# emolch/kiwi

Hardware: AMD Instinct MI355X
Metric: trial-source misfit evals/s (higher is better)
Workload: dtype f32

## Files before the change

### kiwi_amd/csrc/kiwi_accum.hip

```cpp
#include "kiwi_accum_api.hpp"

#if KIWI_ARITH == 0
#define KIWI_ARITH_NS exact
#elif KIWI_ARITH == 1
#define KIWI_ARITH_NS fused
#else
#error "KIWI_ARITH: 0 (exact) or 1 (fused)"
#endif

namespace kiwi {
namespace KIWI_ARITH_NS {

#include "kiwi_accum.inc"

#define KIWI_COMMON_ARGS a.G, a.span, a.pitch, a.recs, a.cent_ofs, a.isrc0, a.nrec, a.recv, a.syn, a.syn_stride

#if KIWI_FAMILY == 1
void launch_direct(const AccumArgs &a, dim3 grid)
{
    if (a.ng == 10) hipLaunchKernelGGL(accumulate_kernel<10>, grid, dim3(256), 0, a.stream, KIWI_COMMON_ARGS, a.synrow);
    else            hipLaunchKernelGGL(accumulate_kernel<8>, grid, dim3(256), 0, a.stream, KIWI_COMMON_ARGS, a.synrow);
}
#endif

// ... 22 lines not shown
    } else {
        if (T == 64) grouped_t<8, 64>(a, grid, ntiles, runs, pairsel, mate, mate4);
        else if (T == 128) grouped_t<8, 128>(a, grid, ntiles, runs, pairsel, mate, mate4);
        else grouped_t<8, 256>(a, grid, ntiles, runs, pairsel, mate, mate4);
    }
}
#endif

#if KIWI_FAMILY == 3
template <int NG, int NS, bool COMPACT, bool PLAN>
static void multi_t(const AccumArgs &a, dim3 grid, int ntiles, const int *mate, const int *wider)
{
    if (a.fuse) hipLaunchKernelGGL((accumulate_multi_kernel<NG, true, NS, COMPACT, PLAN>), grid, dim3(256), 0, a.stream, KIWI_COMMON_ARGS, ntiles, a.tab, a.coefs, a.fp,
                                   a.pairflag, mate, wider, a.plan, a.plan_ofs);
    else        hipLaunchKernelGGL((accumulate_multi_kernel<NG, false, NS, COMPACT, PLAN>), grid, dim3(256), 0, a.stream, KIWI_COMMON_ARGS, ntiles, a.tab, a.coefs, a.fp,
                                   a.pairflag, mate, wider, a.plan, a.plan_ofs);
}
template <int NG, int NS>
static void multi_c(const AccumArgs &a, dim3 grid, int ntiles, const int *mate, const int *wider)
{
    if (a.compact && a.plan) multi_t<NG, NS, true, true>(a, grid, ntiles, mate, wider);
    else if (a.compact) multi_t<NG, NS, true, false>(a, grid, ntiles, mate, wider);
    else multi_t<NG, NS, false, false>(a, grid, ntiles, mate, wider);
}
void launch_multi(const AccumArgs &a, dim3 grid, int NS, int ntiles, const int *mate, const int *wider)
{
    if (a.ng == 10) { if (NS == 4) multi_c<10, 4>(a, grid, ntiles, mate, wider); else multi_c<10, 2>(a, grid, ntiles, mate, wider); }
    else            { if (NS == 4) multi_c<8, 4>(a, grid, ntiles, mate, wider); else multi_c<8, 2>(a, grid, ntiles, mate, wider); }
}
void launch_multi_plan(const AccumArgs &a, int NS, int ngroups, const int *mate, const int *wider, PlanSrc *plan)
{
    const dim3 grid((unsigned)ngroups, (unsigned)((a.nrec + 63) / 64));
    if (NS == 4) hipLaunchKernelGGL(multi_plan_kernel<4>, grid, dim3(64), 0, a.stream, a.recs, a.cent_ofs, a.isrc0, a.nrec, a.recv, a.tab, a.pairflag, mate, wider,
                                    a.plan_ofs, (int4 *)plan);
    else         hipLaunchKernelGGL(multi_plan_kernel<2>, grid, dim3(64), 0, a.stream, a.recs, a.cent_ofs, a.isrc0, a.nrec, a.recv, a.tab, a.pairflag, mate, wider,
                                    a.plan_ofs, (int4 *)plan);
}
#endif

#if KIWI_FAMILY == 4
template <int NG, bool COMPACT>
static void cell_t(const AccumArgs &a, dim3 grid, int ntiles, bool per_wave)
{
#define KIWI_C(KERNEL) hipLaunchKernelGGL(KERNEL, grid, dim3(256), 0, a.stream, KIWI_COMMON_ARGS, ntiles, a.tab, a.coefs, a.fp, a.pairflag, a.synrow, \
                                          a.fam_ofs, a.fam_list)
    if (per_wave) { if (a.fuse) KIWI_C((accumulate_cellw_kernel<NG, true, COMPACT>)); else KIWI_C((accumulate_cellw_kernel<NG, false, COMPACT>)); }
    else          { if (a.fuse) KIWI_C((accumulate_cell_kernel<NG, 256, 2, 0, true, COMPACT>)); else KIWI_C((accumulate_cell_kernel<NG, 256, 2, 0, false, COMPACT>)); }
#undef KIWI_C
}
template <int NG>
static void cell_c(const AccumArgs &a, dim3 grid, int ntiles, bool per_wave)
{
    if (a.compact) cell_t<NG, true>(a, grid, ntiles, per_wave); else cell_t<NG, false>(a, grid, ntiles, per_wave);
}
void launch_cell(const AccumArgs &a, dim3 grid, int ntiles) { if (a.ng == 10) cell_c<10>(a, grid, ntiles, false); else cell_c<8>(a, grid, ntiles, false); }
void launch_cellw(const AccumArgs &a, dim3 grid, int ntiles) { if (a.ng == 10) cell_c<10>(a, grid, ntiles, true); else cell_c<8>(a, grid, ntiles, true); }
int cellw_range() { return kCellwRange; }
#endif

}
}
```

### kiwi_amd/csrc/kiwi_accum.inc

```


typedef float f4u __attribute__((ext_vector_type(4), aligned(4)));
typedef float f2u __attribute__((ext_vector_type(2), aligned(4)));

#if defined(KIWI_EXPLICIT_FMA)
#ifndef KIWI_CELLW_AHEAD
#define KIWI_CELLW_AHEAD 3
#endif
template <class V> __device__ __forceinline__ V kiwi_mad(V acc, float w, V v)
{
    V ws;
    for (int k = 0; k < (int)(sizeof(V) / sizeof(float)); k++) ws[k] = w;
    return __builtin_elementwise_fma(ws, v, acc);
}
template <class V> __device__ __forceinline__ V kiwi_madv(V acc, V w, V v) { return __builtin_elementwise_fma(w, v, acc); }
#else
template <class V> __device__ __forceinline__ V kiwi_mad(V acc, float w, V v) { return acc + w * v; }
template <class V> __device__ __forceinline__ V kiwi_madv(V acc, V w, V v) { return acc + w * v; }
#endif

typedef int v4i_t __attribute__((ext_vector_type(4)));
typedef int v2i_t __attribute__((ext_vector_type(2)));
__device__ __forceinline__ __amdgpu_buffer_rsrc_t gf_rsrc(const float *base)
{
// ... 788 lines not shown
        if constexpr (i < nH1) {
            t1[0] = t1[0] + c1 * s2a<i>(H); t1[0] = t1[0] + c2 * s2a<i>(L);
            t1[1] = t1[1] + c1 * s2b<i>(H); t1[1] = t1[1] + c2 * s2b<i>(L);
        } else if constexpr (i < nH1 + 2) {
            t2[0] = t2[0] + c1 * s2a<i>(H); t2[0] = t2[0] + c2 * s2a<i>(L);
            t2[1] = t2[1] + c1 * s2b<i>(H); t2[1] = t2[1] + c2 * s2b<i>(L);
        } else {
            dz[0] = dz[0] + c1 * s2a<i>(H); dz[0] = dz[0] + c2 * s2a<i>(L);
            dz[1] = dz[1] + c1 * s2b<i>(H); dz[1] = dz[1] + c2 * s2b<i>(L);
        }
        if constexpr (i == nH1 + 1) {
#pragma unroll
            for (int k = 0; k < 2; k++) {
                if (ROT) {
                    ar1[k] = ar1[k] + cl * t1[k] - sl * t2[k];
                    ar2[k] = ar2[k] + cl * t2[k] + sl * t1[k];
                } else {
                    ar1[k] = t1[k]; ar2[k] = t2[k];
                }
            }
        }
    });
}

template <int NG>
__device__ __forceinline__ typename Set2Sel<NG>::type make_set2(f2v &a0, f2v &a1, f2v &a2, f2v &a3, f2v &a4, f2v &a5, f2v &a6, f2v &a7, f2v &a8, f2v &a9,
                                                                f2v &b0, f2v &b1, f2v &b2, f2v &b3, f2v &b4, f2v &b5, f2v &b6, f2v &b7, f2v &b8, f2v &b9)
{
    if constexpr (NG == 10) return Set2_10{ a0, a1, a2, a3, a4, a5, a6, a7, a8, a9, b0, b1, b2, b3, b4, b5, b6, b7, b8, b9 };
    else return Set2_8{ a0, a1, a2, a3, a4, a5, a6, a7, b0, b1, b2, b3, b4, b5, b6, b7 };
}

#include "kiwi_apply_asm.inc"
__device__ __forceinline__ int coef_warm(const float *p)
{
    int d;
    asm volatile("s_load_dword %0, %1, 0x0\n\ts_load_dword %0, %1, 0x40\n\ts_load_dword %0, %1, 0x80\n\ts_load_dword %0, %1, 0xc0\n\t"
                 "s_load_dword %0, %1, 0x100\n\ts_load_dword %0, %1, 0x140\n\ts_load_dword %0, %1, 0x180\n\ts_load_dword %0, %1, 0x1c0"
                 : "=&s"(d) : "s"(p) : "memory");
    return d;
}
#if KIWI_ARITH == 1
#define KIWI_APPLY_ASM(NGV, KV, RV) apply_group_asm_##NGV##_k##KV##_##RV##_fused
#else
#define KIWI_APPLY_ASM(NGV, KV, RV) apply_group_asm_##NGV##_k##KV##_##RV##_exact
#endif

template <int NG, int T, bool FUSE, bool RUNS, bool COMPACT >
__global__ __launch_bounds__(T) __attribute__((amdgpu_waves_per_eu(3))) void accumulate_grouped_kernel(
    const float *__restrict__ G, const int2 *__restrict__ span, int pitch,
    const GeoRec *__restrict__ recs, const int *__restrict__ cent_ofs, int isrc0, int nrec,
    const RecvDev *__restrict__ recv, float *__restrict__ syn, size_t syn_stride, int ntiles,
    const int *__restrict__ tab, const float *__restrict__ coefs, const int *__restrict__ run_first, FuseParams fp,
    const int *__restrict__ pairflag ,
    int pairsel ,
    const int *__restrict__ mate, const int *__restrict__ mate4 ,
    const int *__restrict__ synrow ,
    const int *__restrict__ fam_ofs, const int *__restrict__ fam_list )
{
    constexpr bool compact = COMPACT;
    constexpr int TILE = 4 * T;
    constexpr int LDS_TILE = TILE + kHalo;
    __shared__ __attribute__((aligned(16))) float tiles[NG][LDS_TILE];
    const int s = RUNS ? run_first[blockIdx.x] : (int)blockIdx.x;
    const int s_end = RUNS ? run_first[blockIdx.x + 1] : s + 1;
    const bool multi = RUNS && s_end - s > 1;
    const int tile = blockIdx.y % ntiles, r = blockIdx.y / ntiles;
    const RecvDev &rv = recv[r];
    if (!rv.enabled) return;
    if (tile * TILE >= rv.wlen) return;
    if (pairsel == 1 && cell_pair(rv, pairflag, s, nrec, r)) return;
    if (pairsel == 3 && (multi_taken_fwd<4>(rv, pairflag, mate4, s, nrec, r) || multi_taken_fwd<2>(rv, pairflag, mate, s, nrec, r))) return;
    if (synrow && !multi && synrow[s] != s) return;
    const int tid = threadIdx.x;
    const int lane = tid & 63;
    const int t_tile0 = rv.wbeg + tile * TILE;
    const int cb = cent_ofs[isrc0], c0 = cent_ofs[isrc0 + s], nc = cent_ofs[isrc0 + s + 1] - c0;
    const GeoRec *__restrict__ rc = recs + ((size_t)(c0 - cb) * nrec + (size_t)r * nc);
// ... 456 lines not shown
#pragma unroll
            for (int s = 0; s < NS; s++)
                if (only < 0 || only == s) one_finish<true>(v[i], tile0 + s * SET, LDS_TILE, comp(i), p, gw[s]);
        }
        if (i + DEPTH < N && (i + DEPTH < N - 1 || last_ok)) issue(i + DEPTH);
    }
    if (whalo) {
#pragma unroll
        for (int s = 0; s < NS; s++)
            if (only < 0 || only == s) halo_finish<true>(hact, hv, tile0 + s * SET, LDS_TILE, hig, hph, gw[s]);
    }
}


__device__ __forceinline__ int smax_u(int a, int b) { int r; asm("s_max_i32 %0, %1, %2" : "=s"(r) : "s"(a), "s"(b) : "scc"); return r; }
__device__ __forceinline__ int smin_u(int a, int b) { int r; asm("s_min_i32 %0, %1, %2" : "=s"(r) : "s"(a), "s"(b) : "scc"); return r; }

template <int NS>
__device__ __forceinline__ bool multi_taken(const RecvDev &rv, const int *__restrict__ pairflag, const int *__restrict__ mate,
                                            int s, int nrec, int r)
{
    if (!mate) return false;
    const int a = s - s % NS;
    if (!mate[a / NS] || !rv.need_h || !rv.has_d) return false;
    int f = 0;
#pragma unroll
    for (int i = 0; i < NS; i++) f |= pairflag[(size_t)(a + i) * nrec + r];
    return f == 0;
}

template <int NS>
__global__ __launch_bounds__(64) void multi_plan_kernel(const GeoRec *__restrict__ recs, const int *__restrict__ cent_ofs, int isrc0, int nrec,
    const RecvDev *__restrict__ recv, const int *__restrict__ off4, const int *__restrict__ pairflag, const int *__restrict__ mate,
    const int *__restrict__ mate_wider, const int *__restrict__ plan_ofs, int4 *__restrict__ plan)
{
    constexpr int TILE = 1024 / NS, LDS_TILE = TILE + kHalo;
    const int k = (int)blockIdx.x, s0 = NS * k, r = (int)(blockIdx.y * 64 + threadIdx.x);
    if (r >= nrec) return;
    const RecvDev &rv = recv[r];
    if (!rv.enabled) return;
    if (!multi_taken<NS>(rv, pairflag, mate, s0, nrec, r)) return;
    if constexpr (NS == 2) { if (multi_taken<4>(rv, pairflag, mate_wider, s0, nrec, r)) return; }
    const int cb = cent_ofs[isrc0];
    const int nc = cent_ofs[isrc0 + s0 + 1] - cent_ofs[isrc0 + s0];
    const size_t pbeg = (size_t)plan_ofs[k], pend = (size_t)plan_ofs[k + 1];
    size_t pi = pbeg + (size_t)r;
    for (int c = 0; c < nc && pi < pend; pi += (size_t)nrec) {
        const GeoRec *h[NS];
        int smaxs[NS], smins[NS], npos = 0;
        bool shared = true, same_rows = true;
#pragma unroll
        for (int i = 0; i < NS; i++) {
            h[i] = recs + ((size_t)(cent_ofs[isrc0 + s0 + i] - cb) * nrec + (size_t)r * nc + c);
            smaxs[i] = h[i]->ishift + ((h[i]->pad >> 8) & 0xff);
            smins[i] = h[i]->ishift - ((h[i]->pad >> 16) & 0xff);
            npos = max(npos, TILE + (smaxs[i] - smins[i]) + 8);
            if (i > 0) {
                same_rows = same_rows && h[i]->row[0] == h[0]->row[0] && h[i]->row[1] == h[0]->row[1] && h[i]->row[2] == h[0]->row[2] && h[i]->row[3] == h[0]->row[3];
                shared = shared && smaxs[i] == smaxs[0];
            }
        }
        shared = shared && same_rows;
        if (same_rows && !shared) {
            int smax_c = smaxs[0], smin_c = smins[0];
#pragma unroll
            for (int i = 1; i < NS; i++) { smax_c = max(smax_c, smaxs[i]); smin_c = min(smin_c, smins[i]); }
            if (TILE + (smax_c - smin_c) + 8 <= LDS_TILE) {
                shared = true;
                npos = TILE + (smax_c - smin_c) + 8;
#pragma unroll
                for (int i = 0; i < NS; i++) smaxs[i] = smax_c;
            }
        }
        const int glen = h[0]->pad & 0xff;
        int4 *__restrict__ out = plan + pi * (kPlanStride / 16);
#pragma unroll
        for (int i = 0; i < NS; i++) {
            const int4 o = *(const int4 *)(off4 + ((size_t)(cent_ofs[isrc0 + s0 + i] - cb) * nrec + (size_t)r * nc + c) * 4);
            const int head = (h[i]->flags & 0xffff) | (glen << 16) | ((shared ? 1 : 0) << 23) | ((npos - TILE) << 24);
            out[4 * i + 0] = make_int4(h[i]->row[0], h[i]->row[1], h[i]->row[2], h[i]->row[3]);
            out[4 * i + 1] = o;
            out[4 * i + 2] = make_int4(__float_as_int(h[i]->w[0]), __float_as_int(h[i]->w[1]), __float_as_int(h[i]->w[2]), __float_as_int(h[i]->w[3]));
            out[4 * i + 3] = make_int4(smaxs[i], head, __float_as_int(h[i]->cl), __float_as_int(h[i]->sl));
        }
        if (glen < 1) break;
        c += glen;
    }
}

typedef const __attribute__((address_space(4))) v4i_t *plan_cptr;
template <int NS>
__device__ __forceinline__ int plan_warm(size_t p)
{
    int d;
    if constexpr (NS == 4)
        asm volatile("s_load_dword %0, %1, 0x0\n\ts_load_dword %0, %1, 0x40\n\ts_load_dword %0, %1, 0x80\n\ts_load_dword %0, %1, 0xc0" : "=&s"(d) : "s"(p) : "memory");
    else
        asm volatile("s_load_dword %0, %1, 0x0\n\ts_load_dword %0, %1, 0x40" : "=&s"(d) : "s"(p) : "memory");
    return d;
}

template <int NG, bool FUSE, int NS, bool COMPACT ,
          bool PLAN >
__global__ __launch_bounds__(256) __attribute__((amdgpu_waves_per_eu(3))) void accumulate_multi_kernel(
    const float *__restrict__ G, const int2 *__restrict__ span, int pitch,
    const GeoRec *__restrict__ recs, const int *__restrict__ cent_ofs, int isrc0, int nrec,
    const RecvDev *__restrict__ recv, float *__restrict__ syn, size_t syn_stride, int ntiles,
    const int *__restrict__ tab, const float *__restrict__ coefs, FuseParams fp, const int *__restrict__ pairflag, const int *__restrict__ mate,
    const int *__restrict__ mate_wider ,
    const PlanSrc *__restrict__ plan, const int *__restrict__ plan_ofs )
{
    constexpr bool compact = COMPACT;
    static_assert(NS == 2 || NS == 4, "sources per workgroup");
    static_assert(!PLAN || COMPACT, "plans hold compact descriptors");
    constexpr int TILE = 1024 / NS, LDS_TILE = TILE + kHalo, K = LDS_TILE / 64, WPS = 4 / NS;
    constexpr int SET = multi_set_stride<NG, NS>();
    __shared__ __attribute__((aligned(16))) float tiles[NS * SET];
// ... 94 lines not shown
            }
        }
        }
        const int glen = PLAN ? glen_p : (g[0].pad & 0xff);
        const int cend = c + glen;
        int smax = smaxs[0];
        if constexpr (PLAN) smax = plan4(64 * sh + 48).x;
        else {
#pragma unroll
            for (int i = 1; i < NS; i++) if (sh == i) smax = smaxs[i];
        }
        int flags = 0, ishv = 0, warm_ = 0, pwarm_ = 0;
        float gcl = 0.f, gsl = 0.f;
        const float *__restrict__ coef_grp = nullptr;
        auto shadow = [&]() {
            if constexpr (PLAN) {
#pragma unroll
                for (int i = 0; i < NS; i++) {
                    const v4i_t w = plan4(64 * i + 32);
                    g[i].w[0] = __int_as_float(w.x); g[i].w[1] = __int_as_float(w.y); g[i].w[2] = __int_as_float(w.z); g[i].w[3] = __int_as_float(w.w);
                }
                const v4i_t me = plan4(64 * sh + 48);
                flags = me.y & 0xffff; gcl = __int_as_float(me.z); gsl = __int_as_float(me.w);
                if (c + glen < nc) pwarm_ = plan_warm<NS>(pcur + (size_t)(unsigned)pstep);
            } else {
#pragma unroll
            for (int i = 0; i < NS; i++) { g[i].w[0] = REC_F(cur[i], 4); g[i].w[1] = REC_F(cur[i], 5); g[i].w[2] = REC_F(cur[i], 6); g[i].w[3] = REC_F(cur[i], 7); }
            int curme = cur[0];
#pragma unroll
            for (int i = 1; i < NS; i++) if (sh == i) curme = cur[i];
            flags = REC_I(curme, 18);
            gcl = REC_F(curme, 16); gsl = REC_F(curme, 17);
            }
            if (lane < glen) ishv = rc[c + lane].ishift;
            const size_t crow = (base_me + c) * kCoefLine;
            const unsigned clo = __builtin_amdgcn_readfirstlane((unsigned)crow), chi = __builtin_amdgcn_readfirstlane((unsigned)(crow >> 32));
            coef_grp = coefs + (((size_t)chi << 32) | clo);
            if constexpr (NG == 10) warm_ = coef_warm(coef_grp);
        };
        auto noshadow = []() {};
#define KIWI_MULTI_BUILD(DESC, I0, ONLY, NPOS, SHADOW) do { \
            const int jb_ = t_tile0 - smaxs[I0] - 1;       \
            const float *__restrict__ Gg = G + (size_t)g[I0].row[0] * (size_t)pitch; \
            const bool fast = (DESC).fast(jb_, LDS_TILE, pitch, lane, NG); \
            const bool hact = hq < 16 * NG && hph < (NPOS); \
            const bool whalo = __builtin_amdgcn_ballot_w64(hact) != 0ull; \
            if (fast) multi_build<NG, true, NS>(&tiles[0], wv, lane, tid, jb_, Gg, pitch, DESC, g, ONLY, hact, whalo, hig, hph, SHADOW); \
            else      multi_build<NG, false, NS>(&tiles[0], wv, lane, tid, jb_, Gg, pitch, DESC, g, ONLY, hact, whalo, hig, hph, SHADOW); } while (0)
        __builtin_amdgcn_s_setprio(1);
        if constexpr (PLAN) {
            if (shared) KIWI_MULTI_BUILD(dp, 0, -1, npos, shadow);
            else {
                KIWI_MULTI_BUILD(dp, 0, 0, npos, shadow);
#pragma unroll
                for (int i = 1; i < NS; i++) {
                    const v4i_t rw = plan4(64 * i), of = plan4(64 * i + 16);
                    smaxs[i] = plan4(64 * i + 48).x;
                    g[i].row[0] = rw.x;
                    const DescPlan di{ { 0, (rw.y - rw.x) * pitch, (rw.z - rw.x) * pitch, (rw.w - rw.x) * pitch }, { of.x, of.y, of.z, of.w }, pitch, hoff };
                    KIWI_MULTI_BUILD(di, i, i, npos, noshadow);
                }
            }
            asm volatile("" :: "s"(pwarm_));
            pcur += (size_t)(unsigned)pstep;
        } else {
        if (shared) KIWI_MULTI_BUILD((DescLanes{ ta, tb }), 0, -1, npos, shadow);
        else {
            KIWI_MULTI_BUILD((DescLanes{ ta, tb }), 0, 0, npos, shadow);
#pragma unroll
            for (int i = 1; i < NS; i++) {
                int tai, tbi;
                if constexpr (compact) desc_expand(off4_load(tab_of(i), c, lane), cur[i], lane, pitch, tai, tbi);
                else { tai = tab_of(i)[(size_t)c * 128 + lane]; tbi = tab_of(i)[(size_t)c * 128 + 64 + lane]; }
                g[i].row[0] = REC_I(cur[i], 0);
                KIWI_MULTI_BUILD((DescLanes{ tai, tbi }), i, i, npos, noshadow);
            }
        }
#pragma unroll
        for (int i = 0; i < NS; i++) cur[i] = rec_load(recs_of(i), cend, nc, lane);
        if (cend < nc) {
            if constexpr (compact) ta = off4_load(tab_of(0), cend, lane);
            else { ta = tab_of(0)[(size_t)cend * 128 + lane]; tb = tab_of(0)[(size_t)cend * 128 + 64 + lane]; }
        }
        }
#undef KIWI_MULTI_BUILD
        __syncthreads();
        __builtin_amdgcn_s_setprio(0);
        {
            const unsigned abase = (unsigned)(size_t)(lds_cfp)&tiles[sh * SET + u0];
            if constexpr (NG == 10 || NG == 8) {
                asm volatile("" :: "s"(warm_));
                const float gcl_u = __int_as_float(__builtin_amdgcn_readfirstlane(__float_as_int(gcl))), gsl_u = __int_as_float(__builtin_amdgcn_readfirstlane(__float_as_int(gsl)));
                const size_t cg_ = (size_t)coef_grp;
                const float *__restrict__ coef_u = (const float *)(((size_t)(unsigned)__builtin_amdgcn_readfirstlane((int)(cg_ >> 32)) << 32) | (unsigned)__builtin_amdgcn_readfirstlane((int)cg_));
                const int n = cend - c;
#define KIWI_ASM_ARGS ar1[0], ar1[1], ar2[0], ar2[1], dz[0], dz[1], abase, ishv, smax, n, coef_u, gcl_u, gsl_u
                if constexpr (NG == 10) {
                    if (flags & 2) { if constexpr (K == 5) KIWI_APPLY_ASM(10, 5, rot)(KIWI_ASM_ARGS); else KIWI_APPLY_ASM(10, 9, rot)(KIWI_ASM_ARGS); }
                    else           { if constexpr (K == 5) KIWI_APPLY_ASM(10, 5, plain)(KIWI_ASM_ARGS); else KIWI_APPLY_ASM(10, 9, plain)(KIWI_ASM_ARGS); }
                } else {
                    if (flags & 2) { if constexpr (K == 5) KIWI_APPLY_ASM(8, 5, rot)(KIWI_ASM_ARGS); else KIWI_APPLY_ASM(8, 9, rot)(KIWI_ASM_ARGS); }
                    else           { if constexpr (K == 5) KIWI_APPLY_ASM(8, 5, plain)(KIWI_ASM_ARGS); else KIWI_APPLY_ASM(8, 9, plain)(KIWI_ASM_ARGS); }
                }
#undef KIWI_ASM_ARGS
            } else {
            int cc = c, eprev = 0;
            bool have = false;
#define KIWI_C2STEP(LL, HH, RV, CC) do { \
                const int e = smax - __builtin_amdgcn_readlane(ishv, (CC) - c);        \
                const int d = have ? eprev - e : 0x7fff; \
                carry2_apply<NG, RV, K>(ar1, ar2, dz, LL, HH, abase + 4u * (unsigned)e, d, d, coef_grp + (size_t)((CC) - c) * kCoefLine, gcl, gsl); \
                have = true; eprev = e; } while (0)
            if (flags & 2) {
                set2_dead(X); set2_dead(Y);
                for (; cc + 1 < cend; cc += 2) { KIWI_C2STEP(X, Y, true, cc); KIWI_C2STEP(Y, X, true, cc + 1); }
                if (cc < cend) KIWI_C2STEP(X, Y, true, cc);
            } else {
                set2_dead(X); set2_dead(Y);
                for (; cc + 1 < cend; cc += 2) { KIWI_C2STEP(X, Y, false, cc); KIWI_C2STEP(Y, X, false, cc + 1); }
                if (cc < cend) KIWI_C2STEP(X, Y, false, cc);
            }
#undef KIWI_C2STEP
            }
        }
        c = cend;
    }
    {
        const int js = s0 + sh;
        const int tl = tile * TILE + u0;
        if (!FUSE && tl >= rv.wlen) return;
        float *__restrict__ so = syn + (size_t)js * syn_stride + tl;
        float mom = 0.f;
        if constexpr (FUSE) mom = fp.moment[fp.isrc0 + js];
        const bool whole = tile * TILE + TILE <= rv.wlen;
        for (int k = 0; k < rv.ncomp; k++) {
            f2v o01, o23;
            out4(rv.comp[k], rv.sign[k], rv.cl0, rv.sl0, ar1, ar2, dz, o01, o23);
// ... 585 lines not shown
```

### kiwi_amd/csrc/kiwi_accum_api.hpp

```cpp
#pragma once
#include "kiwi_common.hpp"

namespace kiwi {

struct AccumArgs {
    hipStream_t stream;
    int ng;
    bool fuse;
    const float *G; const int2 *span; int pitch;
    const GeoRec *recs; const int *cent_ofs; int isrc0, nrec;
    const RecvDev *recv; float *syn; size_t syn_stride;
    const int *tab; const float *coefs; FuseParams fp;
    const int *pairflag, *synrow, *fam_ofs, *fam_list;
    int compact;
    const PlanSrc *plan = nullptr;
    const int *plan_ofs = nullptr;
};

#define KIWI_ACCUM_LAUNCHERS                                                                                                      \
                                                                 \
    void launch_direct(const AccumArgs &a, dim3 grid);                                                                            \
                  \
    void launch_grouped(const AccumArgs &a, dim3 grid, int T, int ntiles, const int *runs, int pairsel, const int *mate,          \
                        const int *mate4);                                                                                        \
                                                     \
    void launch_multi(const AccumArgs &a, dim3 grid, int NS, int ntiles, const int *mate, const int *mate_wider);                \
                \
    void launch_multi_plan(const AccumArgs &a, int NS, int ngroups, const int *mate, const int *mate_wider, PlanSrc *plan);      \
        \
    void launch_cell(const AccumArgs &a, dim3 grid, int ntiles);                                                                  \
    void launch_cellw(const AccumArgs &a, dim3 grid, int ntiles);                                                                 \
                               \
    int cellw_range();

namespace exact { KIWI_ACCUM_LAUNCHERS }
namespace fused { KIWI_ACCUM_LAUNCHERS }
#undef KIWI_ACCUM_LAUNCHERS

}
```

### kiwi_amd/csrc/kiwi_common.hpp

```cpp
#pragma once
#include <hip/hip_runtime.h>
#include <type_traits>

namespace kiwi {

constexpr int kRowPad = 32;
constexpr int kTile = 1024;
constexpr int kMaxComp = 5;
constexpr int kHalo = 64;
constexpr int kMaxGroup = 64;

struct GeoRec {
    int   row[4];
    float w[4];
    int   ishift;
    float wfrac;
    float f[6];
    float cl, sl;
    int   flags;
    int   pad;
};
static_assert(sizeof(GeoRec) == 80, "GeoRec layout");

struct GfMeta {
// ... 36 lines not shown
    int ntrans_max;
    int fl_lo, fl_ns, refxofs;
    int untapered, rf0, rf1, vertical;
    int spankind;
};

struct FftPair {
    long long fft_ofs;
    long long spec_ofs;
    int ntrans;
    int specofs;
    int filtofs;
    int slot;
};
static_assert(sizeof(FftPair) == 32, "FftPair layout");

struct ShakeRec {
    int slot[3];
    int np;
    int untapered;
    int rec;
};

constexpr int kCoefLine = 20;
struct PlanSrc {
    int   row[4];
    int   o[4];
    float w[4];
    int   smax;
    int   head;
    float cl, sl;
};
static_assert(sizeof(PlanSrc) == 64, "PlanSrc layout");
constexpr int kPlanStride = 256;
template <int NG> __host__ __device__ constexpr int coef_wl(int a) { return 2 * a; }
template <int NG> __host__ __device__ constexpr int coef_wr(int a) { return 2 * a + 1; }

constexpr int kSpanInts = 8;
__device__ __forceinline__ void strip_span(const int *__restrict__ sp, int kind, int &lo, int &hi)
{
    if (kind == 3) { lo = sp[4]; hi = sp[5]; return; }
    if (kind == 0) { lo = sp[0]; hi = sp[1]; return; }
    if (kind == 1) { lo = sp[2]; hi = sp[3]; return; }
    lo = min(sp[0], sp[2]); hi = max(sp[1], sp[3]);
}

struct EvalParams {
    int bilinear, xus, zus;
    int nrec;
    int isrc0;
    int cellmode;
    int nogaps;
};

__device__ __forceinline__ bool cell_pair(const RecvDev &rv, const int *__restrict__ pairflag, int s, int nrec, int r)
{
    return rv.need_h && rv.has_d && !(pairflag[(size_t)s * nrec + r] & 3);
}

template <int NS>
__device__ __forceinline__ bool multi_taken_fwd(const RecvDev &rv, const int *__restrict__ pairflag, const int *__restrict__ mate,
                                                int s, int nrec, int r)
{
    if (!mate) return false;
    const int a = s - s % NS;
    if (!mate[a / NS] || !rv.need_h || !rv.has_d) return false;
// ... 36 lines not shown
```

### kiwi_amd/csrc/kiwi_hip.hip

```cpp
#include "../../include/kiwi_hip.h"
#include "kiwi_host.hpp"
#include "kiwi_host_eikonal.hpp"
#include "kiwi_host_lm.hpp"
#include "kiwi_geometry.hpp"
#include "kiwi_misfit.hpp"
#include "kiwi_accum_api.hpp"
#include "kiwi_fmm_device.hpp"

#include <hip/hip_runtime.h>
#include <hipfft/hipfft.h>
#include <algorithm>
#include <array>
#include <map>
#include <tuple>
#include <cstdio>
#include <cstdlib>
#include <cstring>
#include <string>
#include <vector>
#include <stdexcept>
#include <omp.h>
#include <chrono>
#include <condition_variable>
#include <deque>
// ... 140 lines not shown
    std::vector<RecvDev> recv_h;
    std::vector<float> norm_h;
    std::vector<float> reft_h;
    DevBuf<RecvDev> recv_d;
    DevBuf<CompDev> comps_d;
    DevBuf<float> reft_d, tw_d, norm_d;
    DevBuf<int> recfirst_d;
    int max_wlen = 0;

    int nsrc = 0;
    std::vector<int> cent_ofs;
    float max_risetime = 0.f;
    DevBuf<float> cent_d, moment_d, risetime_d;
    DevBuf<int> centofs_d;
    std::vector<int> src_status;
    bool any_failed = false;
    DevBuf<int> status_d;
    std::vector<int> same_as;
    bool any_same = false;
    DevBuf<int> synrow_d, famofs_d, famlist_d;
    int dedupe_enabled = 1;
    std::vector<unsigned long long> geo_hash;
    std::vector<kiwi_hip_ctx *> mates;
    int cpu_share = 1;
    std::vector<unsigned long long> struct_hash;
    std::vector<int> ngroups;
    std::vector<unsigned char> group_lens;
    std::vector<int> first_shift;
    std::vector<float> src_ends;
    DevBuf<int> mate_d, mate4_d;
    DevBuf<int> planofs_d;
    DevBuf<int4> plan_d;
    int multi_plan = 1;
    int duo = 4;
    std::vector<char> single_group;
    DevBuf<int> runfirst_d;
    int share_runs = 1, max_run = 64;
    int fuse_enabled = 1;
    bool fuse_now = false;
    DevBuf<double> fusepart_d;

    DevBuf<float> misfit_d, global_d;
    DevBuf<GeoRec> recs_d;
    DevBuf<int> tab_d;
    DevBuf<int> off4_d;
    DevBuf<float> coef_d;
    DevBuf<int> pairflag_d;
    DevBuf<float> syn_d, proc_d;
    bool floating = false;
    int max_ns = 1;
    DevBuf<float> refx_d, vt_d, partial_d;
    DevBuf<int> fshift_d;
    int last_isrc0 = 0, last_nsrc = 0, last_chunk0 = 0, last_chunkn = 0;
    std::vector<char> evaluated;
    int last_proc_which = 0;
    int group_threads_env = 0;
    int group_threads = 128;
    int accum_mode = 0;
    int cell_mode = -1;
    int cell_wave = 1;
    int arith = KIWI_ARITH_EXACT;
    double points_per_centroid = 0.0;
    int keep_which = 0;
    int proc_chunk0 = 0, proc_chunkn = 0, proc_which_held = 0;
    size_t chunk_bytes_limit = (size_t)16 << 30;
    float outer_ms[3] = { 0.f, 0.f, 0.f };
// ... 908 lines not shown
                            c->plan_d.ensure((np + 1) * (kPlanStride / 16), &c->dev_bytes);
                            HIPCHECK(hipMemcpyAsync(c->planofs_d.p, po, (n4 + n2 + 2) * sizeof(int), hipMemcpyHostToDevice, c->stream));
                            if (std::getenv("KIWI_HIP_POISON")) HIPCHECK(hipMemsetAsync(c->plan_d.p, 0x7f, (np + 1) * kPlanStride, c->stream));
                            planned = true;
                        }
                    }
                    HIPCHECK(hipEventRecord(c->mate_event, c->stream));
                }
            }
            const int ntiles_q = (c->max_wlen + 255) / 256;
            dim3 ggrid(gx, (unsigned)(ntiles * nrec));
            dim3 dgrid((unsigned)((nsrc + 1) / 2), (unsigned)(ntiles_p * nrec)), qgrid((unsigned)((nsrc + 3) / 4), (unsigned)(ntiles_q * nrec));
            dim3 cgrid((unsigned)nsrc, (unsigned)(ntiles_c * nrec));
            if (fuse) {
                const int nparts = cell ? std::max(ntiles * (T / 64), ntiles_c * (Tc / 64)) : (duo ? std::max({ ntiles * (T / 64), ntiles_p * 2, ntiles_q }) : ntiles * (T / 64));
                c->fusepart_d.ensure((size_t)nsrc * c->nmis * nparts, &c->dev_bytes);
                if (cell || duo) HIPCHECK(hipMemsetAsync(c->fusepart_d.p, 0, (size_t)nsrc * c->nmis * nparts * sizeof(double), c->stream));
                aa.fp = FuseParams{ c->reft_d.p, c->tw_d.p, c->moment_d.p, c->fusepart_d.p, c->method, c->syn_factor, c->nmis, nparts, isrc0 };
                fuse_nparts = nparts;
            }
            fuse_T = T; fuse_tile = 4 * T; fuse_ntiles = ntiles; fuse_all = cell || duo;
            aa.pairflag = (cell || duo) ? c->pairflag_d.p : (const int *)nullptr;
            if (cell) {
                static const bool cell_fused = [] { const char *e = std::getenv("KIWI_HIP_CELL_FUSED"); return !e || std::atoi(e) != 0; }();
                if (c->cell_wave) { if (fusedar && cell_fused) fused::launch_cellw(aa, cgrid, ntiles_c); else exact::launch_cellw(aa, cgrid, ntiles_c); }
                else exact::launch_cell(aa, cgrid, ntiles_c);
            }
            const int *m2p = any2 ? c->mate_d.p : (const int *)nullptr, *m4p = any4 ? c->mate4_d.p : (const int *)nullptr;
            AccumArgs aa4 = aa, aa2 = aa;
            if (planned) {
                const size_t n4 = (size_t)(nsrc + 3) / 4;
                aa4.plan = (const PlanSrc *)c->plan_d.p; aa4.plan_ofs = c->planofs_d.p;
                aa2.plan = (const PlanSrc *)(c->plan_d.p + plan_n4 * (kPlanStride / 16)); aa2.plan_ofs = c->planofs_d.p + n4 + 1;
                if (any4) { if (fusedar) fused::launch_multi_plan(aa4, 4, (int)qgrid.x, m4p, nullptr, (PlanSrc *)aa4.plan); else exact::launch_multi_plan(aa4, 4, (int)qgrid.x, m4p, nullptr, (PlanSrc *)aa4.plan); }
                if (any2) { if (fusedar) fused::launch_multi_plan(aa2, 2, (int)dgrid.x, m2p, m4p, (PlanSrc *)aa2.plan); else exact::launch_multi_plan(aa2, 2, (int)dgrid.x, m2p, m4p, (PlanSrc *)aa2.plan); }
            }
            if (any4) { if (fusedar) fused::launch_multi(aa4, qgrid, 4, ntiles_q, m4p, nullptr); else exact::launch_multi(aa4, qgrid, 4, ntiles_q, m4p, nullptr); }
            if (any2) { if (fusedar) fused::launch_multi(aa2, dgrid, 2, ntiles_p, m2p, m4p); else exact::launch_multi(aa2, dgrid, 2, ntiles_p, m2p, m4p); }
            const int pairsel = cell ? 1 : (duo ? 3 : 0);
            if (fusedar) fused::launch_grouped(aa, ggrid, T, ntiles, runs, pairsel, m2p, m4p);
            else         exact::launch_grouped(aa, ggrid, T, ntiles, runs, pairsel, m2p, m4p);
        }
    }
    record(c, 1, e2);
    if (c->any_untapered) {
        c->synspan_d.ensure((size_t)nsrc * c->nmis * 2, &c->dev_bytes);
        hipLaunchKernelGGL(synspan_kernel, dim3((unsigned)c->nmis, (unsigned)nsrc), dim3(256), 0, c->stream, c->syn_d.p, c->syn_stride, c->comps_d.p,
                           c->risetime_d.p + isrc0, c->gm.dt, c->nmis, spansrc, nrec, synrow, c->synspan_d.p);
    }
    if (c->untapered_fft) {
        const size_t np = (size_t)nsrc * c->nmis;
        c->ntr_d.ensure(np, &c->dev_bytes);
        pin_ensure(c->ntr_pin, c->ntr_pin_n, np);
        hipLaunchKernelGGL(fft_size_kernel, dim3((unsigned)((np + 255) / 256)), dim3(256), 0, c->stream, spansrc, c->comps_d.p, c->nmis,
                           nsrc, nrec, c->risetime_d.p + isrc0, c->gm.dt, c->ntr_d.p, (const int *)c->synspan_d.p);
        HIPCHECK(hipMemcpyAsync(c->ntr_pin, c->ntr_d.p, np * sizeof(int), hipMemcpyDeviceToHost, c->stream));
        HIPCHECK(hipEventRecord(c->size_event, c->stream));
    }
    if (c->fft_needed) layout_fft_chunk(c, isrc0, nsrc);
    {
        const bool spectral = (c->method == KIWI_AMPSPEC_L2NORM || c->method == KIWI_AMPSPEC_L1NORM);
        const int fl_method = c->method == KIWI_FLOATING_L2NORM ? KIWI_L2NORM : KIWI_L1NORM;
        const int td_method = spectral ? KIWI_L2NORM : (c->floating ? fl_method : c->method);
        const int fft_mode = !c->fft_needed ? 0 : (spectral ? 3 : 1);
        MisfitParams mp{ td_method, c->gm.dt, c->syn_factor, c->nmis, isrc0, proc_which == 3 ? 2 : proc_which, fft_mode, nsrc,
                         c->floating ? 1 : 0 };
        if (c->floating) {
            c->vt_d.ensure((size_t)nsrc * c->syn_stride, &c->dev_bytes);
// ... 170 lines not shown
#pragma unroll
        for (int k = 0; k < 8; k++) v[k] = __builtin_nontemporal_load(p + i + 256 * k);
#pragma unroll
        for (int k = 0; k < 8; k++) { x ^= v[k].x; y ^= v[k].y; z ^= v[k].z; w ^= v[k].w; }
    }
    for (; i < b; i += 256) { const read_u4 v = p[i]; x ^= v.x; y ^= v.y; z ^= v.z; w ^= v.w; }
    if ((x ^ y ^ z ^ w) == 0x9e3779b9u) sink[blockIdx.x] = x;
}

extern "C" {

int kiwi_hip_init(int device, kiwi_hip_ctx **out)
{
    kmp_set_blocktime(0);
    kiwi_hip_ctx *c = nullptr;
    try {
        int ndev = 0;
        hipError_t e = hipGetDeviceCount(&ndev);
        if (e != hipSuccess || ndev <= 0)
            return fail(nullptr, std::string("no HIP device available: ") + hipGetErrorString(e));
        if (device < 0 || device >= ndev) return fail(nullptr, "device index out of range");
        HIPCHECK(hipSetDevice(device));
        c = new kiwi_hip_ctx();
        c->device = device;
        HIPCHECK(hipStreamCreateWithFlags(&c->stream, hipStreamNonBlocking));
        if (const char *m = std::getenv("KIWI_HIP_GROUP_THREADS")) {
            const int v = std::atoi(m);
            if (v == 64 || v == 128 || v == 256) { c->group_threads = v; c->group_threads_env = 1; }
        }
        if (const char *m = std::getenv("KIWI_HIP_ACCUM")) c->accum_mode = (std::strcmp(m, "direct") == 0) ? 1 : 0;
        if (const char *m = std::getenv("KIWI_HIP_FUSE")) c->fuse_enabled = std::atoi(m);
        if (const char *m = std::getenv("KIWI_HIP_DUO")) { const int v = std::atoi(m); c->duo = v >= 4 ? 4 : (v >= 1 ? 2 : 0); }
        if (const char *m = std::getenv("KIWI_HIP_MULTI_PLAN")) c->multi_plan = std::atoi(m) ? 1 : 0;
        if (const char *m = std::getenv("KIWI_HIP_CELL")) c->cell_mode = std::atoi(m) ? 1 : 0;
        if (const char *m = std::getenv("KIWI_HIP_DEDUPE")) c->dedupe_enabled = std::atoi(m);
        if (const char *m = std::getenv("KIWI_HIP_FUSED_FFT")) c->fused_fft = std::atoi(m) != 0;
        if (const char *m = std::getenv("KIWI_HIP_ARITH")) {
            if (std::strcmp(m, "fused") == 0 || std::strcmp(m, "fma") == 0) c->arith = KIWI_ARITH_FUSED;
            else if (std::strcmp(m, "exact") != 0) throw std::runtime_error("KIWI_HIP_ARITH: exact or fused");
        }
        if (const char *m = std::getenv("KIWI_HIP_CELL_WAVE")) c->cell_wave = std::atoi(m) ? 1 : 0;
        if (const char *m = std::getenv("KIWI_HIP_COMPACT")) c->compact = std::atoi(m) ? 1 : 0;
        if (const char *m = std::getenv("KIWI_HIP_CHUNK_MB")) {
            const long v = std::atol(m);
            if (v > 0) c->chunk_bytes_limit = (size_t)v << 20;
        }
        if (const char *m = std::getenv("KIWI_HIP_EIK_DEVICE")) c->eik_solver = std::atoi(m) ? 1 : 0;
        if (const char *m = std::getenv("KIWI_HIP_RUNS")) {
            const int v = std::atoi(m);
            c->share_runs = v != 0;
            if (v > 1) c->max_run = v;
        }
        *out = c;
        return 0;
    } catch (const std::exception &e) {
        delete c;
        return fail(nullptr, e.what());
    }
}

int kiwi_hip_init_multi(int ndev_wanted, kiwi_hip_ctx **out)
{
    if (!out) return fail(nullptr, "null argument");
    *out = nullptr;
    int ndev = 0;
    hipError_t e = hipGetDeviceCount(&ndev);
// ... 2321 lines not shown
```

### kiwi_amd/lib.py

```python
import ctypes as C
import os
import sys
import re
import subprocess

HERE = os.path.dirname(os.path.abspath(__file__))
LIB_PATH = os.environ.get("KIWI_HIP_LIB", os.path.join(HERE, "libkiwi_hip.so"))
HEADER = os.path.join(os.path.dirname(HERE), "include", "kiwi_hip.h")

c_float_p = C.POINTER(C.c_float)
c_int_p = C.POINTER(C.c_int)
c_double_p = C.POINTER(C.c_double)


class KiwiHipError(RuntimeError):
    """A C-ABI call returned non-zero; the message is the library's last error
    (the reference's '<cmd>: nok >' line, minimizer.f90:1689-1696)."""


RESIDUAL_FN = C.CFUNCTYPE(C.c_int, C.c_void_p, C.c_int, C.c_int, C.c_int, C.POINTER(C.c_float), C.POINTER(C.c_float))


def build(force=False):
    if force and os.path.exists(LIB_PATH):
        os.remove(LIB_PATH)
    subprocess.check_call(["make", "-s", "-C", os.path.join(HERE, "csrc")])
    return LIB_PATH


def declared_symbols():
    txt = open(HEADER).read()
    return sorted(set(re.findall(r"\b(kiwi_hip_[a-z_0-9]+)\s*\(", txt)))


_lib = None


def load():
    global _lib
    if _lib is not None:
        return _lib
    if not os.path.exists(LIB_PATH):
        raise KiwiHipError("%s not built -- run `python -c 'import __graft_entry__ as g; g.build()'` "
                           "or `make -C kiwi_amd/csrc`" % LIB_PATH)
    import importlib.util
    if "torch" not in sys.modules and os.environ.get("KIWI_HIP_WITHOUT_TORCH", "0") != "1" and importlib.util.find_spec("torch") is not None:
        try:
            import torch
        except Exception:
            pass
    L = C.CDLL(LIB_PATH)
    vp = C.c_void_p
    sig = {
        "kiwi_hip_init": [C.c_int, C.POINTER(vp)],
        "kiwi_hip_init_multi": [C.c_int, C.POINTER(vp)],
        "kiwi_hip_ndevices": [vp, c_int_p],
        "kiwi_hip_set_arithmetic": [vp, C.c_int],
        "kiwi_hip_get_arithmetic": [vp, c_int_p],
        "kiwi_hip_destroy": [vp],
# ... 136 lines not shown
```

Before: 36870.

## Mark regular-shift plan groups and use specialized asm apply path

The plan kernel now detects centroid groups whose per-column ishift values increase by exactly one, and encodes the starting offset and a regular flag into the plan header. The multi accumulate kernel then skips the per-lane ishift load for such groups and dispatches to new plan-specific asm apply routines that derive shifts from the header. A debug-only counter of regular plans is added. This aims to cut ishift gathers and index arithmetic in the inner apply loop, at the cost of more plan-building work and extra code variants. The new asm include file is not shown, and the build now passes the Python path to make, which suggests the asm is generated by a script.

```diff
diff --git a/kiwi_amd/csrc/kiwi_accum.hip b/kiwi_amd/csrc/kiwi_accum.hip
--- a/kiwi_amd/csrc/kiwi_accum.hip
+++ b/kiwi_amd/csrc/kiwi_accum.hip
@@ -78,9 +78,9 @@
 {
     const dim3 grid((unsigned)ngroups, (unsigned)((a.nrec + 63) / 64));
     if (NS == 4) hipLaunchKernelGGL(multi_plan_kernel<4>, grid, dim3(64), 0, a.stream, a.recs, a.cent_ofs, a.isrc0, a.nrec, a.recv, a.tab, a.pairflag, mate, wider,
-                                    a.plan_ofs, (int4 *)plan);
+                                    a.plan_ofs, (int4 *)plan, a.plan_regular, a.plan_count);
     else         hipLaunchKernelGGL(multi_plan_kernel<2>, grid, dim3(64), 0, a.stream, a.recs, a.cent_ofs, a.isrc0, a.nrec, a.recv, a.tab, a.pairflag, mate, wider,
-                                    a.plan_ofs, (int4 *)plan);
+                                    a.plan_ofs, (int4 *)plan, a.plan_regular, a.plan_count);
 }
 #endif
 
diff --git a/kiwi_amd/csrc/kiwi_accum.inc b/kiwi_amd/csrc/kiwi_accum.inc
--- a/kiwi_amd/csrc/kiwi_accum.inc
+++ b/kiwi_amd/csrc/kiwi_accum.inc
@@ -844,6 +844,7 @@
 }
 
 #include "kiwi_apply_asm.inc"
+#include "kiwi_apply_plan_asm.inc"
 __device__ __forceinline__ int coef_warm(const float *p)
 {
     int d;
@@ -854,8 +855,10 @@
 }
 #if KIWI_ARITH == 1
 #define KIWI_APPLY_ASM(NGV, KV, RV) apply_group_asm_##NGV##_k##KV##_##RV##_fused
+#define KIWI_APPLY_PLAN(NGV, KV, RV) apply_plan_asm_##NGV##_k##KV##_##RV##_fused
 #else
 #define KIWI_APPLY_ASM(NGV, KV, RV) apply_group_asm_##NGV##_k##KV##_##RV##_exact
+#define KIWI_APPLY_PLAN(NGV, KV, RV) apply_plan_asm_##NGV##_k##KV##_##RV##_exact
 #endif
 
 template <int NG, int T, bool FUSE, bool RUNS, bool COMPACT >
@@ -1378,7 +1381,8 @@
 template <int NS>
 __global__ __launch_bounds__(64) void multi_plan_kernel(const GeoRec *__restrict__ recs, const int *__restrict__ cent_ofs, int isrc0, int nrec,
     const RecvDev *__restrict__ recv, const int *__restrict__ off4, const int *__restrict__ pairflag, const int *__restrict__ mate,
-    const int *__restrict__ mate_wider, const int *__restrict__ plan_ofs, int4 *__restrict__ plan)
+    const int *__restrict__ mate_wider, const int *__restrict__ plan_ofs, int4 *__restrict__ plan,
+    int regular_on , unsigned *__restrict__ count )
 {
     constexpr int TILE = 1024 / NS, LDS_TILE = TILE + kHalo;
     const int k = (int)blockIdx.x, s0 = NS * k, r = (int)(blockIdx.y * 64 + threadIdx.x);
@@ -1420,15 +1424,21 @@
         }
         const int glen = h[0]->pad & 0xff;
         int4 *__restrict__ out = plan + pi * (kPlanStride / 16);
+        unsigned nreg = 0;
 #pragma unroll
         for (int i = 0; i < NS; i++) {
             const int4 o = *(const int4 *)(off4 + ((size_t)(cent_ofs[isrc0 + s0 + i] - cb) * nrec + (size_t)r * nc + c) * 4);
-            const int head = (h[i]->flags & 0xffff) | (glen << 16) | ((shared ? 1 : 0) << 23) | ((npos - TILE) << 24);
+            const int e0 = smaxs[i] - h[i]->ishift;
+            bool regular = regular_on != 0 && e0 >= 0 && e0 <= kPlanE0Mask;
+            for (int j = 1; j < glen && c + j < nc; j++) regular = regular && h[i][j].ishift == h[i][j - 1].ishift + 1;
+            nreg += regular ? 1u : 0u;
+            const int head = (h[i]->flags & 0xffff) | (regular ? (e0 << kPlanE0Shift) | kPlanRegularBit : 0) | (glen << 16) | ((shared ? 1 : 0) << 23) | ((npos - TILE) << 24);
             out[4 * i + 0] = make_int4(h[i]->row[0], h[i]->row[1], h[i]->row[2], h[i]->row[3]);
             out[4 * i + 1] = o;
             out[4 * i + 2] = make_int4(__float_as_int(h[i]->w[0]), __float_as_int(h[i]->w[1]), __float_as_int(h[i]->w[2]), __float_as_int(h[i]->w[3]));
             out[4 * i + 3] = make_int4(smaxs[i], head, __float_as_int(h[i]->cl), __float_as_int(h[i]->sl));
         }
+        if (count) { atomicAdd(count, (unsigned)NS); atomicAdd(count + 1, nreg); }
         if (glen < 1) break;
         c += glen;
     }
@@ -1589,7 +1599,7 @@
             flags = REC_I(curme, 18);
             gcl = REC_F(curme, 16); gsl = REC_F(curme, 17);
             }
-            if (lane < glen) ishv = rc[c + lane].ishift;
+            if (!(PLAN && (flags & kPlanRegularBit))) { if (lane < glen) ishv = rc[c + lane].ishift; }
             const size_t crow = (base_me + c) * kCoefLine;
             const unsigned clo = __builtin_amdgcn_readfirstlane((unsigned)crow), chi = __builtin_amdgcn_readfirstlane((unsigned)(crow >> 32));
             coef_grp = coefs + (((size_t)chi << 32) | clo);
@@ -1652,6 +1662,17 @@
                 const float *__restrict__ coef_u = (const float *)(((size_t)(unsigned)__builtin_amdgcn_readfirstlane((int)(cg_ >> 32)) << 32) | (unsigned)__builtin_amdgcn_readfirstlane((int)cg_));
                 const int n = cend - c;
 #define KIWI_ASM_ARGS ar1[0], ar1[1], ar2[0], ar2[1], dz[0], dz[1], abase, ishv, smax, n, coef_u, gcl_u, gsl_u
+#define KIWI_PLAN_ARGS ar1[0], ar1[1], ar2[0], ar2[1], dz[0], dz[1], abase, ishv, smax, n, coef_u, gcl_u, gsl_u, head_u
+                if constexpr (PLAN) {
+                    const int head_u = __builtin_amdgcn_readfirstlane(flags);
+                    if constexpr (NG == 10) {
+                        if (flags & 2) { if constexpr (K == 5) KIWI_APPLY_PLAN(10, 5, rot)(KIWI_PLAN_ARGS); else KIWI_APPLY_PLAN(10, 9, rot)(KIWI_PLAN_ARGS); }
+                        else           { if constexpr (K == 5) KIWI_APPLY_PLAN(10, 5, plain)(KIWI_PLAN_ARGS); else KIWI_APPLY_PLAN(10, 9, plain)(KIWI_PLAN_ARGS); }
+                    } else {
+                        if (flags & 2) { if constexpr (K == 5) KIWI_APPLY_PLAN(8, 5, rot)(KIWI_PLAN_ARGS); else KIWI_APPLY_PLAN(8, 9, rot)(KIWI_PLAN_ARGS); }
+                        else           { if constexpr (K == 5) KIWI_APPLY_PLAN(8, 5, plain)(KIWI_PLAN_ARGS); else KIWI_APPLY_PLAN(8, 9, plain)(KIWI_PLAN_ARGS); }
+                    }
+                } else
                 if constexpr (NG == 10) {
                     if (flags & 2) { if constexpr (K == 5) KIWI_APPLY_ASM(10, 5, rot)(KIWI_ASM_ARGS); else KIWI_APPLY_ASM(10, 9, rot)(KIWI_ASM_ARGS); }
                     else           { if constexpr (K == 5) KIWI_APPLY_ASM(10, 5, plain)(KIWI_ASM_ARGS); else KIWI_APPLY_ASM(10, 9, plain)(KIWI_ASM_ARGS); }
@@ -1660,6 +1681,7 @@
                     else           { if constexpr (K == 5) KIWI_APPLY_ASM(8, 5, plain)(KIWI_ASM_ARGS); else KIWI_APPLY_ASM(8, 9, plain)(KIWI_ASM_ARGS); }
                 }
 #undef KIWI_ASM_ARGS
+#undef KIWI_PLAN_ARGS
             } else {
             int cc = c, eprev = 0;
             bool have = false;
diff --git a/kiwi_amd/csrc/kiwi_accum_api.hpp b/kiwi_amd/csrc/kiwi_accum_api.hpp
--- a/kiwi_amd/csrc/kiwi_accum_api.hpp
+++ b/kiwi_amd/csrc/kiwi_accum_api.hpp
@@ -15,6 +15,8 @@
     int compact;
     const PlanSrc *plan = nullptr;
     const int *plan_ofs = nullptr;
+    int plan_regular = 1;
+    unsigned *plan_count = nullptr;
 };
 
 #define KIWI_ACCUM_LAUNCHERS                                                                                                      \
diff --git a/kiwi_amd/csrc/kiwi_common.hpp b/kiwi_amd/csrc/kiwi_common.hpp
--- a/kiwi_amd/csrc/kiwi_common.hpp
+++ b/kiwi_amd/csrc/kiwi_common.hpp
@@ -92,6 +92,7 @@
     float cl, sl;
 };
 static_assert(sizeof(PlanSrc) == 64, "PlanSrc layout");
+constexpr int kPlanE0Shift = 4, kPlanE0Mask = 0x7f, kPlanRegularBit = 1 << 11;
 constexpr int kPlanStride = 256;
 template <int NG> __host__ __device__ constexpr int coef_wl(int a) { return 2 * a; }
 template <int NG> __host__ __device__ constexpr int coef_wr(int a) { return 2 * a + 1; }
diff --git a/kiwi_amd/csrc/kiwi_hip.hip b/kiwi_amd/csrc/kiwi_hip.hip
--- a/kiwi_amd/csrc/kiwi_hip.hip
+++ b/kiwi_amd/csrc/kiwi_hip.hip
@@ -196,6 +196,8 @@
     DevBuf<int> planofs_d;
     DevBuf<int4> plan_d;
     int multi_plan = 1;
+    int multi_regular = 1;
+    DevBuf<unsigned> plancount_d;
     int duo = 4;
     std::vector<char> single_group;
     DevBuf<int> runfirst_d;
@@ -1170,8 +1172,21 @@
                 const size_t n4 = (size_t)(nsrc + 3) / 4;
                 aa4.plan = (const PlanSrc *)c->plan_d.p; aa4.plan_ofs = c->planofs_d.p;
                 aa2.plan = (const PlanSrc *)(c->plan_d.p + plan_n4 * (kPlanStride / 16)); aa2.plan_ofs = c->planofs_d.p + n4 + 1;
+                aa4.plan_regular = aa2.plan_regular = c->multi_regular;
+                const bool count_plans = std::getenv("KIWI_HIP_DEBUG") != nullptr;
+                if (count_plans) {
+                    c->plancount_d.ensure(2, &c->dev_bytes);
+                    HIPCHECK(hipMemsetAsync(c->plancount_d.p, 0, 2 * sizeof(unsigned), c->stream));
+                    aa4.plan_count = aa2.plan_count = c->plancount_d.p;
+                }
                 if (any4) { if (fusedar) fused::launch_multi_plan(aa4, 4, (int)qgrid.x, m4p, nullptr, (PlanSrc *)aa4.plan); else exact::launch_multi_plan(aa4, 4, (int)qgrid.x, m4p, nullptr, (PlanSrc *)aa4.plan); }
                 if (any2) { if (fusedar) fused::launch_multi_plan(aa2, 2, (int)dgrid.x, m2p, m4p, (PlanSrc *)aa2.plan); else exact::launch_multi_plan(aa2, 2, (int)dgrid.x, m2p, m4p, (PlanSrc *)aa2.plan); }
+                if (count_plans) {
+                    unsigned cnt[2] = { 0u, 0u };
+                    HIPCHECK(hipMemcpyAsync(cnt, c->plancount_d.p, sizeof(cnt), hipMemcpyDeviceToHost, c->stream));
+                    HIPCHECK(hipStreamSynchronize(c->stream));
+                    std::fprintf(stderr, "[kiwi_hip] multi plans: %u of a (source, centroid group, receiver), %u regular\n", cnt[0], cnt[1]);
+                }
             }
             if (any4) { if (fusedar) fused::launch_multi(aa4, qgrid, 4, ntiles_q, m4p, nullptr); else exact::launch_multi(aa4, qgrid, 4, ntiles_q, m4p, nullptr); }
             if (any2) { if (fusedar) fused::launch_multi(aa2, dgrid, 2, ntiles_p, m2p, m4p); else exact::launch_multi(aa2, dgrid, 2, ntiles_p, m2p, m4p); }
@@ -1408,6 +1423,7 @@
         if (const char *m = std::getenv("KIWI_HIP_FUSE")) c->fuse_enabled = std::atoi(m);
         if (const char *m = std::getenv("KIWI_HIP_DUO")) { const int v = std::atoi(m); c->duo = v >= 4 ? 4 : (v >= 1 ? 2 : 0); }
         if (const char *m = std::getenv("KIWI_HIP_MULTI_PLAN")) c->multi_plan = std::atoi(m) ? 1 : 0;
+        if (const char *m = std::getenv("KIWI_HIP_MULTI_REGULAR")) c->multi_regular = std::atoi(m) ? 1 : 0;
         if (const char *m = std::getenv("KIWI_HIP_CELL")) c->cell_mode = std::atoi(m) ? 1 : 0;
         if (const char *m = std::getenv("KIWI_HIP_DEDUPE")) c->dedupe_enabled = std::atoi(m);
         if (const char *m = std::getenv("KIWI_HIP_FUSED_FFT")) c->fused_fft = std::atoi(m) != 0;
diff --git a/kiwi_amd/lib.py b/kiwi_amd/lib.py
--- a/kiwi_amd/lib.py
+++ b/kiwi_amd/lib.py
@@ -24,7 +24,7 @@
 def build(force=False):
     if force and os.path.exists(LIB_PATH):
         os.remove(LIB_PATH)
-    subprocess.check_call(["make", "-s", "-C", os.path.join(HERE, "csrc")])
+    subprocess.check_call(["make", "-s", "-C", os.path.join(HERE, "csrc"), "PYTHON=" + sys.executable])
     return LIB_PATH
 
 
```

New measurement: 37400 (median of 6 runs). +1.4%, better.
